# dev-wei/recman

Hardware: AMD Instinct MI355X
Metric: examples/sec fwd+bwd, Criteo-shape batch 65536; % HBM and MFMA roofline (higher is better)
Workload: dtype f32; 1 GPU; deepfm (BASELINE configs[1]); batch_per_gpu=65536, batch_all_gpus=65536, sparse_fields=26, rows_per_field=1000001, dense_fields=13, emb_dim=16, indices=uniform, table_row_loads=cached (rm_deepfm_step), row_gradient_stores=cached (as in fit(): the optimizer step gathers them next), optimizer_step=excluded, matrix_arithmetic=f32 MFMA (v_mfma_f32_16x16x4_f32), fp32 accumulate, hipgraph=True, table=single GPU

## Files before the change

recman_amd/build.py:

```python
import glob
import os
import shutil
import subprocess
import sys

CSRC = os.path.join(os.path.dirname(os.path.abspath(__file__)), "csrc")
LIB = os.path.join(CSRC, "librecman_hip.so")
ARCH = "gfx950"


def sources():
    return sorted(glob.glob(os.path.join(CSRC, "*.hip")))


def _stale():
    if not os.path.exists(LIB):
        return True
    t = os.path.getmtime(LIB)
    deps = sources() + glob.glob(os.path.join(CSRC, "*.h")) + glob.glob(
        os.path.join(CSRC, "..", "..", "include", "*.h"))
    return any(os.path.getmtime(p) > t for p in deps)


def hipcc():
    exe = shutil.which("hipcc") or "/opt/rocm/bin/hipcc"
    if not os.path.exists(exe):
        raise RuntimeError("hipcc not found: cannot build librecman_hip.so")
    return exe


def clean_experiments(verbose=True):
    for p in glob.glob(os.path.join(CSRC, "librecman_*.so")):
        if os.path.abspath(p) != os.path.abspath(LIB):
            if verbose:
                print(f"[build] removing stray experiment build {p}", flush=True)
            os.remove(p)


def build(force=False, verbose=True, extra_flags=(), out=None, only=None):
    clean_experiments(verbose)
    if out is None and not force and not _stale():
        return LIB
    if out is not None:
        if only:
            build(force=False, verbose=verbose)
        return _build_variant(out, extra_flags, verbose, only)
    objs = []
    procs = []
    for src in sources():
        obj = src[:-4] + ".o"
        cmd = [hipcc(), "-O3", "-std=c++17", f"--offload-arch={ARCH}", "-fPIC", "-c", src, "-o", obj,
               "-Wall", "-Wno-unused-function", *extra_flags]
        if verbose:
            print(" ".join(cmd), flush=True)
        procs.append((src, subprocess.Popen(cmd)))
        objs.append(obj)
    for src, p in procs:
        if p.wait() != 0:
            raise RuntimeError(f"hipcc failed on {src}")
    cmd = [hipcc(), "-shared", "-fPIC", f"--offload-arch={ARCH}", *objs, "-o", LIB]
    if verbose:
        print(" ".join(cmd), flush=True)
    subprocess.check_call(cmd)
    return LIB


def _build_variant(out, extra_flags, verbose, only=None):
    out = os.path.abspath(out)
    os.makedirs(os.path.dirname(out), exist_ok=True)
    tag = os.path.splitext(os.path.basename(out))[0]
    objs, procs = [], []
    for src in sources():
        if only and os.path.basename(src)[:-4] not in only:
            objs.append(src[:-4] + ".o")
            continue
        obj = os.path.join(os.path.dirname(out), f"{tag}_{os.path.basename(src)[:-4]}.o")
        cmd = [hipcc(), "-O3", "-std=c++17", f"--offload-arch={ARCH}", "-fPIC", "-c", src, "-o", obj,
               "-Wall", "-Wno-unused-function", *extra_flags]
        if verbose:
            print(" ".join(cmd), flush=True)
        procs.append((src, subprocess.Popen(cmd)))
        objs.append(obj)
    for src, p in procs:
        if p.wait() != 0:
            raise RuntimeError(f"hipcc failed on {src}")
    subprocess.check_call([hipcc(), "-shared", "-fPIC", f"--offload-arch={ARCH}", *objs, "-o", out])
    return out


if __name__ == "__main__":
    argv = sys.argv[1:]
    out = argv[argv.index("--out") + 1] if "--out" in argv else None
    flags = [a for a in argv if a.startswith("-D")]
    only = argv[argv.index("--only") + 1].split(",") if "--only" in argv else None
    print(build(force="--force" in argv, out=out, extra_flags=flags, only=only))
```

recman_amd/csrc/step.hip:

```cpp
#include "mlp_internal.h"
#include "rm_common.h"

namespace {

typedef float f32x4 __attribute__((ext_vector_type(4)));
typedef unsigned u32x4 __attribute__((ext_vector_type(4)));
typedef __amdgpu_buffer_rsrc_t rsrc_t;

constexpr int kWorkers = 7;
constexpr int kSlots = 4;
constexpr int kMaxF = 26;
constexpr int kRing = 3;
constexpr int kSlotB = 1024;
constexpr int kXBufB = kMaxF * kSlotB;
constexpr int kPartH = 0, kPartS = 2048, kPartQ = 3072, kPartSd = 3328, kPartB = 3584;
constexpr int kLDT = 36;
constexpr int kPubDh = 0, kPubDT = 2048, kPubGS = kPubDT + 16 * kLDT * 4, kPubG = kPubGS + 1024, kPubB = kPubG + 256;
constexpr int oX = 0;
constexpr int oDense = oX + kRing * kXBufB;
constexpr int oJunk = oDense + 4 * kSlotB;
constexpr int oPart = oJunk + kSlotB;
constexpr int oPub = oPart + 2 * kWorkers * kPartB;
constexpr int kRowB = 28 * 64;
constexpr int oRow = oPub + 2 * kPubB;
constexpr int oHT = oRow + 2 * kRowB;
constexpr int oD1T = oHT + 16 * 32 * 4;
constexpr int oY = oD1T + 16 * 32 * 4;
constexpr int oW1 = oY + 4 * 16 * 4;
constexpr int oPar = oW1 + 32 * 32 * 4;
constexpr int kParB0 = 0, kParB1 = 128, kParWo = 256, kParWd = 384, kParFo = 448;
constexpr int kLdsBytes = oPar + 448 + 28 * 4;
static_assert(kLdsBytes <= 160 * 1024, "LDS map exceeds a CU");

#ifndef RM_STEP_ABL
#define RM_STEP_ABL 0
#endif
#ifdef RM_STEP_STAMP
__device__ unsigned long long rm_step_stamp_buf[256 * 8 * 8];
#define ST_NOW() __builtin_amdgcn_s_memtime()
#define ST_DECL unsigned long long st_acc[8] = {0, 0, 0, 0, 0, 0, 0, 0}, st_t = ST_NOW(), st_t0 = st_t
#define ST_ADD(i) { const unsigned long long st_n = ST_NOW(); st_acc[i] += st_n - st_t; st_t = st_n; }
#define ST_FLUSH(wv) if (lane == 0 && blockIdx.x < 256) { st_acc[7] = ST_NOW() - st_t0; for (int i_ = 0; i_ < 8; ++i_) rm_step_stamp_buf[(blockIdx.x * 8 + (wv)) * 8 + i_] = st_acc[i_]; }
#else
#define ST_DECL
#define ST_ADD(i)
#define ST_FLUSH(wv)
#endif

struct StepArgs {
  const int64_t *idx, *field_off;
  const char *table;
  int64_t row_bytes;
  const float *dense;
  const int64_t *y;
  const float *y_f;
  const float *W0, *b0, *W1, *b1, *w_out, *w0_out, *lin_wd, *lin_w0;
  int F, Dn, H0, H1, act, task, Kp;
  float grad_scale;
  int64_t B;
  float *d_rows, *logit, *pred, *dlogit, *dW0_part, *sg_part, *loss_part;
  int packed, out_row_bytes, out_rows;
  const float *lin_mask;
};

__device__ __forceinline__ float act_slope(int act) {
  return act == RM_ACT_RELU ? 0.f : (act == RM_ACT_LEAKY_RELU ? 0.2f : 1.f);
}
__device__ __forceinline__ float actf(float v, float slope) { return v > 0.f ? v : slope * v; }
__device__ __forceinline__ float actg(float o, float slope) { return o > 0.f ? 1.f : slope; }

__device__ __forceinline__ int slot_field(int w, int j) {
  return j < 3 ? 7 * j + w : (w < 3 ? 21 + w : (w > 3 ? 20 + w : -1));
}

__device__ __forceinline__ f32x4 mfma16(float a, float b, f32x4 c) {
  return __builtin_amdgcn_mfma_f32_16x16x4f32(a, b, c, 0, 0, 0);
}
__device__ __forceinline__ f32x4 mfma16w(float a, float b, f32x4 c) {
  if (RM_STEP_ABL & 16) { c.x += a * b; return c; }
  return __builtin_amdgcn_mfma_f32_16x16x4f32(a, b, c, 0, 0, 0);
}

__device__ __forceinline__ int swz(int r) { return ((r >> 3) & 1) * 3; }

template <bool NT>
__device__ __forceinline__ void dma16(const char *src, char *lds_dst) {
  __builtin_amdgcn_global_load_lds((const __attribute__((address_space(1))) void *)src,
                                   (__attribute__((address_space(3))) void *)lds_dst, 16, 0, NT ? 2 : 0);
}

__device__ __forceinline__ void wait_vm(int younger) {
#define RM_WV(N) case N: asm volatile("s_waitcnt vmcnt(" #N ")" ::: "memory"); break;
  switch (younger) {
    RM_WV(24) RM_WV(23) RM_WV(22) RM_WV(21) RM_WV(20) RM_WV(19) RM_WV(18) RM_WV(17) RM_WV(16) RM_WV(15) RM_WV(14) RM_WV(13) RM_WV(12) RM_WV(11) RM_WV(10) RM_WV(9) RM_WV(8) RM_WV(7) RM_WV(6)
    RM_WV(5) RM_WV(4) RM_WV(3) RM_WV(2) RM_WV(1)
    default: asm volatile("s_waitcnt vmcnt(0)" ::: "memory"); break;
  }
#undef RM_WV
}

__device__ __forceinline__ float sum_q(float v) {
  {
    float a = v, c = v;
    asm("s_nop 1\n\tv_permlane16_swap_b32 %0, %1" : "+v"(a), "+v"(c));
    v = a + c;
  }
  {
    float a = v, c = v;
    asm("s_nop 1\n\tv_permlane32_swap_b32 %0, %1" : "+v"(a), "+v"(c));
    v = a + c;
  }
  return v;
}
__device__ __forceinline__ float sum_n(float v) {
#pragma unroll
  for (int o = 1; o < 16; o <<= 1) v += __shfl_xor(v, o, 64);
  return v;
}

template <bool NT, bool NT_OUT, bool PACKED>
__device__ __forceinline__ void step_worker(const StepArgs &a, char *smem, const int w, const int lane, const int T) {
  const int n = lane & 15, q = lane >> 4;
  const int F = a.F, H0 = a.H0, K = 16 * F + a.Dn;
  int fld[kSlots];
  bool sv[kSlots], sx[kSlots];
  float w0f[kSlots][2][4];
  float w0x[kSlots][2][4];
  f32x4 dw[kSlots][2];
#pragma unroll
  for (int j = 0; j < kSlots; ++j) {
    const int f = slot_field(w, j);
    sv[j] = f >= 0 && (f < F || (f == F && a.Dn > 0));
    sx[j] = f >= 0 && f < F;
    fld[j] = sv[j] ? f : 0;
    const int kb = 16 * fld[j];
#pragma unroll
    for (int uh = 0; uh < 2; ++uh) {
#pragma unroll
      for (int e = 0; e < 4; ++e) {
        const int kf = kb + 4 * q + e, uf = 16 * uh + n;
        const bool okf = sv[j] && kf < K && uf < H0;
        const float vf = a.W0[okf ? (int64_t)kf * H0 + uf : 0];
        w0f[j][uh][e] = okf ? vf : 0.f;
        const int kx = kb + n, ux = 16 * uh + 4 * q + e;
        const bool okx = sx[j] && kx < K && ux < H0;
        const float vx = a.W0[okx ? (int64_t)kx * H0 + ux : 0];
        w0x[j][uh][e] = okx ? vx : 0.f;
      }
      dw[j][uh] = f32x4{0.f, 0.f, 0.f, 0.f};
    }
  }
  const int64_t tstride = gridDim.x;
  const int lo_slice = n * 64 + 16 * (q ^ swz(n));
  int lo_col[4];
#pragma unroll
  for (int es = 0; es < 4; ++es) lo_col[es] = (4 * es + q) * 64 + 16 * ((n >> 2) ^ swz(4 * es + q)) + 4 * (n & 3);
  const int lo_row = n * F * 64 + 16 * q;
  auto slot_base = [&](int j, int tile) {
    const int ring = oX + ((tile + 6) % 3) * kXBufB + fld[j] * kSlotB, dn = oDense + (tile & 3) * kSlotB;
    return __builtin_amdgcn_readfirstlane((sx[j] || !sv[j]) ? ring : dn);
  };
  const int piece = 16 * ((lane & 3) ^ swz(lane >> 2));
  const int side_off = 64 + 4 * (lane & 1);
  float sdv[kSlots];
#pragma unroll
  for (int j = 0; j < kSlots; ++j) sdv[j] = 0.f;
  unsigned rp[4][kSlots];
  float lmask[kSlots];
#pragma unroll
  for (int j = 0; j < kSlots; ++j) {
    rp[0][j] = rp[1][j] = rp[2][j] = rp[3][j] = 0;
    lmask[j] = (PACKED && a.lin_mask != nullptr && sx[j]) ? a.lin_mask[fld[j]] : 1.f;
  }
  ST_DECL;
  ST_ADD(0);

  for (int s = -2; s <= T + 1; ++s) {
    const bool hasB = s - 2 >= 0 && s - 2 < T;
    const bool hasD = s + 1 >= 0 && s + 1 < T;
    float side_sum = 0.f;
#pragma unroll
    for (int j = 0; j < kSlots; ++j) side_sum += sx[j] ? sdv[j] : 0.f;
    {
      const int tb = s - 2, td = s + 1;
      const char *pub = smem + oPub + (tb & 1) * kPubB;
      char *xd = smem + oX + ((td + 3) % 3) * kXBufB;
      f32x4 dhB[2], gS, e4[kSlots];
      float dT[2][4], g, col[kSlots][4];
      if (hasB) {
#pragma unroll
        for (int j = 0; j < kSlots; ++j) {
          const char *xs = smem + slot_base(j, tb);
#pragma unroll
          for (int es = 0; es < 4; ++es)
            col[j][es] = *reinterpret_cast<const float *>(xs + lo_col[es]);
          e4[j] = *reinterpret_cast<const f32x4 *>(xs + lo_slice);
        }
#pragma unroll
        for (int uh = 0; uh < 2; ++uh) {
          dhB[uh] = *reinterpret_cast<const f32x4 *>(pub + kPubDh + (uh * 64 + lane) * 16);
#pragma unroll
          for (int es = 0; es < 4; ++es)
            dT[uh][es] = *reinterpret_cast<const float *>(pub + kPubDT + ((4 * es + q) * kLDT + 16 * uh + n) * 4);
        }
        gS = *reinterpret_cast<const f32x4 *>(pub + kPubGS + lane * 16);
        g = *reinterpret_cast<const float *>(pub + kPubG + lane * 4);
      }
      ST_ADD(1);
      unsigned rid[kSlots];
      if (PACKED) {
#pragma unroll
        for (int j = 0; j < kSlots; ++j) {
          rp[3][j] = rp[2][j];
          rp[2][j] = rp[1][j];
          rp[1][j] = rp[0][j];
        }
      }
      if (hasD) {
        const unsigned *rowid = reinterpret_cast<const unsigned *>(smem + oRow + (td & 1) * kRowB);
#pragma unroll
        for (int j = 0; j < kSlots; ++j) {
          rid[j] = rowid[fld[j] * 16 + (lane >> 2)];
          if (PACKED) rp[0][j] = rowid[fld[j] * 16 + n];
        }
      }
      asm volatile("s_waitcnt lgkmcnt(0)" ::: "memory");
      const int64_t ex0 = ((int64_t)blockIdx.x + tb * tstride) * 16;
      const int64_t left = a.B - ex0;
      const int rows_t = left < 16 ? (int)left : 16;
      const rsrc_t rd = PACKED ? __builtin_amdgcn_make_buffer_rsrc(a.d_rows, 0, hasB ? a.out_rows * a.out_row_bytes : 0, 0x00020000)
                               : __builtin_amdgcn_make_buffer_rsrc(a.d_rows + (hasB ? ex0 * F * 16 : 0), 0,
                                                                   hasB ? rows_t * F * 64 : 0, 0x00020000);
      const bool ex_ok = n < rows_t;
      auto store_row = [&](int i, const f32x4 &o) {
        const bool ok = sx[i] && !(RM_STEP_ABL & 2);
        if (PACKED) {
          const int base = (ok && ex_ok) ? (int)rp[3][i] * a.out_row_bytes : 0x7ffffff0 - 64;
          __builtin_amdgcn_raw_buffer_store_b128(__builtin_bit_cast(u32x4, o), rd, base + 16 * q, 0, NT_OUT ? 2 : 0);
          const f32x4 tail = f32x4{g, g * lmask[i], 0.f, 0.f};
          __builtin_amdgcn_raw_buffer_store_b128(__builtin_bit_cast(u32x4, tail), rd, q == 0 ? base + 64 : 0x7ffffff0,
                                                 0, NT_OUT ? 2 : 0);
        } else {
          const int off = lo_row + __builtin_amdgcn_readfirstlane(ok ? fld[i] * 64 : 0x70000000);
          __builtin_amdgcn_raw_buffer_store_b128(__builtin_bit_cast(u32x4, o), rd, off, 0, NT_OUT ? 2 : 0);
        }
      };
      f32x4 acc[kSlots];
#pragma unroll
      for (int j = 0; j < kSlots; ++j) {
        if (hasD) {
          const char *row = a.table + ((RM_STEP_ABL & 4) || !sx[j] ? 0 : (int64_t)rid[j] * a.row_bytes);
          if (!(RM_STEP_ABL & 8)) dma16<NT>(row + piece, sx[j] ? xd + fld[j] * kSlotB : smem + oJunk);
          if (!(RM_STEP_ABL & 1)) sdv[j] = *reinterpret_cast<const float *>(row + side_off);
        }
        __builtin_amdgcn_sched_barrier(0);
        if (hasB) {
          acc[j] = f32x4{0.f, 0.f, 0.f, 0.f};
#pragma unroll
          for (int es = 0; es < 4; ++es) {
            dw[j][0] = mfma16w(col[j][es], dT[0][es], dw[j][0]);
            dw[j][1] = mfma16w(col[j][es], dT[1][es], dw[j][1]);
            acc[j] = mfma16w(w0x[j][0][es], dhB[0][es], acc[j]);
            acc[j] = mfma16w(w0x[j][1][es], dhB[1][es], acc[j]);
          }
        }
        __builtin_amdgcn_sched_barrier(0);
        if (hasB && j > 0) {
          const int i = j - 1;
          f32x4 o;
          o.x = acc[i].x + (gS.x - g * e4[i].x);
          o.y = acc[i].y + (gS.y - g * e4[i].y);
          o.z = acc[i].z + (gS.z - g * e4[i].z);
          o.w = acc[i].w + (gS.w - g * e4[i].w);
          store_row(i, o);
        }
      }
      if (hasB) {
        const int i = kSlots - 1;
        f32x4 o;
        o.x = acc[i].x + (gS.x - g * e4[i].x);
        o.y = acc[i].y + (gS.y - g * e4[i].y);
        o.z = acc[i].z + (gS.z - g * e4[i].z);
        o.w = acc[i].w + (gS.w - g * e4[i].w);
        store_row(i, o);
      }
    }
    ST_ADD(6);
    if (s >= 0 && s < T) {
      constexpr int SP = PACKED ? 2 : 1;
      const int younger = 1 + ((s - 3 >= 0) ? 2 * SP : 0) + 8 * (hasD ? 1 : 0) + 4 * SP * (hasB ? 1 : 0);
      wait_vm(younger);
      ST_ADD(3);
      f32x4 acc0 = f32x4{0.f, 0.f, 0.f, 0.f}, acc1 = acc0, S = acc0, Q = acc0;
      f32x4 x4[kSlots];
#pragma unroll
      for (int j = 0; j < kSlots; ++j) {
        x4[j] = *reinterpret_cast<const f32x4 *>(smem + slot_base(j, s) + lo_slice);
      }
#pragma unroll
      for (int j = 0; j < kSlots; ++j) {
#pragma unroll
        for (int ks = 0; ks < 4; ++ks) {
          acc0 = mfma16w(w0f[j][0][ks], x4[j][ks], acc0);
          acc1 = mfma16w(w0f[j][1][ks], x4[j][ks], acc1);
        }
        const float m = sx[j] ? 1.f : 0.f;
        S += m * x4[j];
        Q += m * (x4[j] * x4[j]);
      }
      char *part = smem + oPart + ((s & 1) * kWorkers + w) * kPartB;
      *reinterpret_cast<f32x4 *>(part + kPartH + lane * 16) = acc0;
      *reinterpret_cast<f32x4 *>(part + kPartH + (64 + lane) * 16) = acc1;
      *reinterpret_cast<f32x4 *>(part + kPartS + lane * 16) = S;
      *reinterpret_cast<float *>(part + kPartQ + lane * 4) = (Q.x + Q.y) + (Q.z + Q.w);
      *reinterpret_cast<float *>(part + kPartSd + lane * 4) = side_sum;
    }
    ST_ADD(4);
    __syncthreads();
    ST_ADD(5);
  }
#pragma unroll
  for (int j = 0; j < kSlots; ++j)
    if (sv[j]) {
#pragma unroll
      for (int uh = 0; uh < 2; ++uh)
#pragma unroll
        for (int i = 0; i < 4; ++i)
          a.dW0_part[((int64_t)blockIdx.x * a.Kp + 16 * fld[j] + 4 * q + i) * 32 + 16 * uh + n] = dw[j][uh][i];
    }
  ST_ADD(0);
  ST_FLUSH(w);
}

__device__ __forceinline__ void step_head(const StepArgs &a, char *smem, const int lane, const int T) {
  const int n = lane & 15, q = lane >> 4;
  const int F = a.F, Dn = a.Dn, H0 = a.H0, H1 = a.H1;
  const float act = act_slope(a.act);
  const int64_t B = a.B, tstride = gridDim.x;
  {
    float *w1s = reinterpret_cast<float *>(smem + oW1);
#pragma unroll
    for (int i = 0; i < 16; ++i) {
      const int e = lane + 64 * i, u = e >> 5, v = e & 31;
      const bool ok = u < H0 && v < H1;
      const float f = a.W1[ok ? u * H1 + v : 0];
      w1s[u * 32 + 4 * ((v >> 2) ^ (u & 7)) + (v & 3)] = ok ? f : 0.f;
    }
    float *par = reinterpret_cast<float *>(smem + oPar);
    if (lane < 32) {
      const float f0 = a.b0[lane < H0 ? lane : 0], f1 = a.b1[lane < H1 ? lane : 0], f2 = a.w_out[lane < H1 ? lane : 0];
      par[kParB0 / 4 + lane] = lane < H0 ? f0 : 0.f;
      par[kParB1 / 4 + lane] = lane < H1 ? f1 : 0.f;
      par[kParWo / 4 + lane] = lane < H1 ? f2 : 0.f;
      const float f3 = a.lin_wd[lane < Dn ? lane : 0];
      if (lane < 16) par[kParWd / 4 + lane] = lane < Dn ? f3 : 0.f;
      if (lane < 28) reinterpret_cast<unsigned *>(par)[kParFo / 4 + lane] = (unsigned)a.field_off[lane < F ? lane : F - 1];
    }
  }
  const float *w1s = reinterpret_cast<const float *>(smem + oW1);
  const char *par = smem + oPar;
  const float w0o = a.w0_out[0], lw0 = a.lin_w0[0];

  f32x4 dW1[2][2];
  float db0[2][4], db1[2][4], dwo[2][4], dxd[4], sg = 0.f, loss_acc = 0.f;
#pragma unroll
  for (int x = 0; x < 2; ++x)
#pragma unroll
    for (int i = 0; i < 4; ++i) {
      dW1[x][0][i] = dW1[x][1][i] = 0.f;
      db0[x][i] = db1[x][i] = dwo[x][i] = 0.f;
    }
#pragma unroll
  for (int i = 0; i < 4; ++i) dxd[i] = 0.f;

  auto ex_of = [&](int t) {
    const int64_t b = ((int64_t)blockIdx.x + t * tstride) * 16 + n;
    return b < B ? b : B - 1;
  };
  unsigned idr[7];
  float dnr[4];
  unsigned yr = 0;
#pragma unroll
  for (int j = 0; j < 7; ++j) idr[j] = 0;
#pragma unroll
  for (int i = 0; i < 4; ++i) dnr[i] = 0.f;
  auto load_ids = [&](int t) {
    const unsigned *p = reinterpret_cast<const unsigned *>(a.idx + ex_of(t) * F);
#pragma unroll
    for (int j = 0; j < 7; ++j) idr[j] = p[2 * (q + 4 * j < F ? q + 4 * j : F - 1)];
  };
  if (T > 0) load_ids(0);
  ST_DECL;
  ST_ADD(0);

  for (int s = -2; s <= T + 1; ++s) {
    if (s - 1 >= 0 && s - 1 < T) {
      const int t = s - 1;
      const int64_t bex = ((int64_t)blockIdx.x + t * tstride) * 16 + n;
      const bool valid = bex < B;
      f32x4 pre[2], S = f32x4{0.f, 0.f, 0.f, 0.f};
      pre[0] = pre[1] = S;
      float ss = 0.f, y1 = 0.f, ls = 0.f;
#pragma unroll
      for (int w = 0; w < kWorkers; ++w) {
        const char *part = smem + oPart + ((t & 1) * kWorkers + w) * kPartB;
        pre[0] += *reinterpret_cast<const f32x4 *>(part + kPartH + lane * 16);
        pre[1] += *reinterpret_cast<const f32x4 *>(part + kPartH + (64 + lane) * 16);
        S += *reinterpret_cast<const f32x4 *>(part + kPartS + lane * 16);
        ss += *reinterpret_cast<const float *>(part + kPartQ + lane * 4);
        const float2 sd = *reinterpret_cast<const float2 *>(part + kPartSd + 16 * n);
        y1 += sd.x;
        ls += sd.y;
        if (w == 3) __builtin_amdgcn_sched_barrier(0);
      }
      const f32x4 dn4 = Dn > 0 ? *reinterpret_cast<const f32x4 *>(smem + oDense + (t & 3) * kSlotB + n * 64 + 16 * (q ^ swz(n)))
                               : f32x4{0.f, 0.f, 0.f, 0.f};
      const f32x4 wdv = *reinterpret_cast<const f32x4 *>(par + kParWd + 16 * q);
      const float fmq = sum_q(S.x * S.x + S.y * S.y + S.z * S.z + S.w * S.w - ss);
      const float lind = sum_q(dn4.x * wdv.x + dn4.y * wdv.y + dn4.z * wdv.z + dn4.w * wdv.w);
      const float fm = y1 + 0.5f * fmq;
      const float lin = ls + lind + lw0;
      const float ty = *reinterpret_cast<const float *>(smem + oY + ((t & 3) * 16 + n) * 4);
      ST_ADD(1);
      float h0[2][4], h1[2][4];
#pragma unroll
      for (int h = 0; h < 2; ++h) {
        const f32x4 b0v = *reinterpret_cast<const f32x4 *>(par + kParB0 + (16 * h + 4 * q) * 4);
#pragma unroll
        for (int i = 0; i < 4; ++i) h0[h][i] = actf(pre[h][i] + b0v[i], act);
        *reinterpret_cast<f32x4 *>(smem + oHT + (n * 32 + 16 * h + 4 * q) * 4) =
            f32x4{h0[h][0], h0[h][1], h0[h][2], h0[h][3]};
      }
      f32x4 acc[2];
      acc[0] = acc[1] = f32x4{0.f, 0.f, 0.f, 0.f};
#pragma unroll
      for (int uh = 0; uh < 2; ++uh)
#pragma unroll
        for (int i = 0; i < 4; ++i) {
          const int u = 16 * uh + 4 * q + i;
          const float a0 = w1s[u * 32 + 4 * ((n >> 2) ^ (u & 7)) + (n & 3)];
          const float a1 = w1s[u * 32 + 4 * ((4 + (n >> 2)) ^ (u & 7)) + (n & 3)];
          acc[0] = mfma16(a0, h0[uh][i], acc[0]);
          acc[1] = mfma16(a1, h0[uh][i], acc[1]);
        }
      float dnn = 0.f;
      f32x4 wov[2];
#pragma unroll
      for (int h = 0; h < 2; ++h) {
        const f32x4 b1v = *reinterpret_cast<const f32x4 *>(par + kParB1 + (16 * h + 4 * q) * 4);
        wov[h] = *reinterpret_cast<const f32x4 *>(par + kParWo + (16 * h + 4 * q) * 4);
#pragma unroll
        for (int i = 0; i < 4; ++i) {
          h1[h][i] = actf(acc[h][i] + b1v[i], act);
          dnn += h1[h][i] * wov[h][i];
        }
      }
      dnn = sum_q(dnn) + w0o;
      float z = 0.f;
      z += lin;
      z += fm;
      z += dnn;
      float p, dz;
      const float lt = rm_loss_point(z, ty, a.task, &p, &dz);
      float gb = dz * (1.0f / (float)B);
      gb *= a.grad_scale;
      gb = valid ? gb : 0.f;
      if (valid && q == 0) {
        a.logit[bex] = z;
        a.pred[bex] = p;
        a.dlogit[bex] = gb;
        loss_acc += lt;
      }
      ST_ADD(2);
      float dh1[2][4], dh0[2][4];
#pragma unroll
      for (int h = 0; h < 2; ++h) {
#pragma unroll
        for (int i = 0; i < 4; ++i) dh1[h][i] = gb * wov[h][i] * actg(h1[h][i], act);
        *reinterpret_cast<f32x4 *>(smem + oD1T + (n * 32 + 16 * h + 4 * q) * 4) =
            f32x4{dh1[h][0], dh1[h][1], dh1[h][2], dh1[h][3]};
      }
      acc[0] = acc[1] = f32x4{0.f, 0.f, 0.f, 0.f};
#pragma unroll
      for (int vh = 0; vh < 2; ++vh) {
        const f32x4 c0 = *reinterpret_cast<const f32x4 *>(w1s + n * 32 + 4 * ((4 * vh + q) ^ (n & 7)));
        const f32x4 c1 = *reinterpret_cast<const f32x4 *>(w1s + (16 + n) * 32 + 4 * ((4 * vh + q) ^ (n & 7)));
#pragma unroll
        for (int i = 0; i < 4; ++i) {
          acc[0] = mfma16(c0[i], dh1[vh][i], acc[0]);
          acc[1] = mfma16(c1[i], dh1[vh][i], acc[1]);
        }
      }
      char *pub = smem + oPub + (t & 1) * kPubB;
#pragma unroll
      for (int h = 0; h < 2; ++h) {
#pragma unroll
        for (int i = 0; i < 4; ++i) dh0[h][i] = acc[h][i] * actg(h0[h][i], act);
        const f32x4 d4 = f32x4{dh0[h][0], dh0[h][1], dh0[h][2], dh0[h][3]};
        *reinterpret_cast<f32x4 *>(pub + kPubDh + (h * 64 + lane) * 16) = d4;
        *reinterpret_cast<f32x4 *>(pub + kPubDT + (n * kLDT + 16 * h + 4 * q) * 4) = d4;
      }
      *reinterpret_cast<f32x4 *>(pub + kPubGS + lane * 16) = f32x4{gb * S.x, gb * S.y, gb * S.z, gb * S.w};
      *reinterpret_cast<float *>(pub + kPubG + lane * 4) = gb;
      ST_ADD(3);
#pragma unroll
      for (int es = 0; es < 4; ++es) {
        float av[2], bv[2];
#pragma unroll
        for (int h = 0; h < 2; ++h) {
          av[h] = *reinterpret_cast<const float *>(smem + oHT + ((4 * es + q) * 32 + 16 * h + n) * 4);
          bv[h] = *reinterpret_cast<const float *>(smem + oD1T + ((4 * es + q) * 32 + 16 * h + n) * 4);
        }
#pragma unroll
        for (int uh = 0; uh < 2; ++uh)
#pragma unroll
          for (int vh = 0; vh < 2; ++vh) dW1[uh][vh] = mfma16(av[uh], bv[vh], dW1[uh][vh]);
      }
#pragma unroll
      for (int h = 0; h < 2; ++h)
#pragma unroll
        for (int i = 0; i < 4; ++i) {
          db0[h][i] += dh0[h][i];
          db1[h][i] += dh1[h][i];
          dwo[h][i] += gb * h1[h][i];
        }
      sg += q == 0 ? gb : 0.f;
      dxd[0] += gb * dn4.x;
      dxd[1] += gb * dn4.y;
      dxd[2] += gb * dn4.z;
      dxd[3] += gb * dn4.w;
    }
    ST_ADD(4);
    if (s + 1 >= 0 && s + 1 < T) {
      const int t = s + 1;
      if (Dn > 0)
        *reinterpret_cast<f32x4 *>(smem + oDense + (t & 3) * kSlotB + n * 64 + 16 * (q ^ swz(n))) =
            f32x4{4 * q + 0 < Dn ? dnr[0] : 0.f, 4 * q + 1 < Dn ? dnr[1] : 0.f, 4 * q + 2 < Dn ? dnr[2] : 0.f,
                  4 * q + 3 < Dn ? dnr[3] : 0.f};
      if (q == 0)
        *reinterpret_cast<float *>(smem + oY + ((t & 3) * 16 + n) * 4) = a.y ? (float)(int)yr : __uint_as_float(yr);
    }
    if (s + 2 < T) {
      unsigned *rowid = reinterpret_cast<unsigned *>(smem + oRow + ((s + 2) & 1) * kRowB);
#pragma unroll
      for (int j = 0; j < 7; ++j)
        rowid[(q + 4 * j) * 16 + n] = idr[j] + *reinterpret_cast<const unsigned *>(par + kParFo + (q + 4 * j) * 4);
    }
    __builtin_amdgcn_sched_barrier(0);
    if (s + 2 >= 0 && s + 2 < T) {
      const int64_t b = ex_of(s + 2);
      if (Dn > 0) {
        const float *dp = a.dense + b * Dn;
#pragma unroll
        for (int i = 0; i < 4; ++i) dnr[i] = dp[4 * q + i < Dn ? 4 * q + i : 0];
      }
      const unsigned *yp = a.y ? reinterpret_cast<const unsigned *>(a.y + b) : reinterpret_cast<const unsigned *>(a.y_f + b);
      yr = *yp;
    }
    if (s + 3 < T) load_ids(s + 3);
    ST_ADD(6);
    __syncthreads();
    ST_ADD(5);
  }

  float *sgp = a.sg_part + (int64_t)blockIdx.x * kRmSgStride;
#pragma unroll
  for (int uh = 0; uh < 2; ++uh)
#pragma unroll
    for (int vh = 0; vh < 2; ++vh)
#pragma unroll
      for (int i = 0; i < 4; ++i) sgp[(16 * uh + 4 * q + i) * 32 + 16 * vh + n] = dW1[uh][vh][i];
#pragma unroll
  for (int h = 0; h < 2; ++h)
#pragma unroll
    for (int i = 0; i < 4; ++i) {
      const float s0 = sum_n(db0[h][i]), s1 = sum_n(db1[h][i]), s2 = sum_n(dwo[h][i]);
      if (n == 0) {
        const int u = 16 * h + 4 * q + i;
        sgp[2 * 1024 + u] = s0;
        sgp[2 * 1024 + 32 + u] = s1;
        sgp[2 * 1024 + 64 + u] = s2;
      }
    }
#pragma unroll
  for (int i = 0; i < 4; ++i) {
    const float sx = sum_n(dxd[i]);
    if (n == 0) sgp[kRmSgDense + 4 * q + i] = sx;
  }
  const float sgt = rm_wave_sum(sg), lst = rm_wave_sum(loss_acc);
  if (lane == 0) {
    sgp[2 * 1024 + 64 + 32] = sgt;
    a.loss_part[blockIdx.x] = lst;
  }
  ST_ADD(0);
  ST_FLUSH(7);
}

template <bool NT, bool NT_OUT, bool PACKED>
__global__ __launch_bounds__(512) void deepfm_step_kernel(StepArgs a) {
  extern __shared__ __attribute__((aligned(16))) char smem[];
  const int lane = threadIdx.x & 63;
  const int wave = __builtin_amdgcn_readfirstlane(threadIdx.x >> 6);
  const int64_t ntiles = (a.B + 15) / 16;
  const int T = (int)((ntiles - blockIdx.x + gridDim.x - 1) / gridDim.x);
#ifndef RM_STEP_PRIO
#define RM_STEP_PRIO 1
#endif
  if (wave < kWorkers) {
    if (RM_STEP_PRIO == 1 && wave >= 4) __builtin_amdgcn_s_setprio(1);
    step_worker<NT, NT_OUT, PACKED>(a, smem, wave, lane, T);
  } else {
    if (RM_STEP_PRIO) __builtin_amdgcn_s_setprio(2);
    step_head(a, smem, lane, T);
  }
}

}

#ifdef RM_STEP_STAMP
extern "C" int rm_debug_step_stamps(unsigned long long *host, int n) {
  return (int)hipMemcpyFromSymbol(host, HIP_SYMBOL(rm_step_stamp_buf), sizeof(unsigned long long) * n);
}
#endif

extern "C" int64_t rm_deepfm_step_workspace(int F, int Dn) {
  const int Kp = ((16 * F + Dn + 63) / 64) * 64;
  return (int64_t)256 * Kp * 32 + (int64_t)256 * kRmSgStride + 256;
}

extern "C" int rm_deepfm_step_supported(int F, int D, int64_t table_ld, int Dn, int NL, const int *H) {
  if (D != 16 || table_ld < 20 || table_ld % 4 != 0 || F < 1 || F > 26 || Dn < 0 || Dn > 16 || NL != 2 || !H) return 0;
  return H[0] >= 1 && H[0] <= 32 && H[1] >= 1 && H[1] <= 32;
}

extern "C" int rm_deepfm_step(const int64_t *idx, const float *table, int64_t table_ld, const int64_t *field_off,
                              const float *dense, int Dn, const int64_t *y, const float *y_f, int64_t B, int F,
                              int D, int NL, const int *H, const float *const *W, const float *const *bias,
                              const float *w_out, const float *w0_out, const float *lin_w_dense,
                              const float *lin_w0, int act, int task, float grad_scale, float *d_rows,
                              float *logit, float *pred, float *dlogit, float *loss, float *const *dW,
                              float *const *db, float *d_w_out, float *d_w0_out, float *d_lin_w_dense,
                              float *d_lin_w0, float *workspace, int64_t packed_rows, const float *lin_field_mask,
                              int flags, rm_stream_t stream) {
  RM_REQUIRE(H && rm_deepfm_step_supported(F, D, table_ld, Dn, NL, H),
             "rm_deepfm_step: needs D = 16, fused rows (table_ld >= 20, a multiple of 4), F <= 26, Dn <= 16 and two "
             "hidden layers of width <= 32");
  RM_REQUIRE(B >= 0, "rm_deepfm_step: B < 0");
  if (B == 0) return RM_OK;
  RM_REQUIRE(idx && table && field_off && (Dn == 0 || (dense && lin_w_dense)) && W && bias && W[0] && W[1] &&
                 bias[0] && bias[1] && w_out && w0_out && lin_w0 && d_rows && logit && pred && dlogit && loss && dW &&
                 dW[0] && dW[1] && workspace,
             "rm_deepfm_step: NULL argument");
  RM_REQUIRE((y != nullptr) != (y_f != nullptr), "rm_deepfm_step: exactly one of y / y_f");
  RM_REQUIRE(task == 0 || task == 1, "rm_deepfm_step: task must be 0 or 1");
  RM_REQUIRE(rm_aligned16(table) && rm_aligned16(d_rows), "rm_deepfm_step: table / d_rows must be 16-byte aligned");
  RM_REQUIRE(packed_rows >= 0 && packed_rows * 80 < (1ll << 31), "rm_deepfm_step: packed_rows out of range");
  const int K = 16 * F + Dn, Kp = ((K + 63) / 64) * 64;
  const int64_t ntiles = (B + 15) / 16;
  const int nblk = rm_grid_cap(ntiles, 256);
  StepArgs a;
  a.idx = idx; a.field_off = field_off; a.table = reinterpret_cast<const char *>(table); a.row_bytes = table_ld * 4;
  a.dense = dense; a.y = y; a.y_f = y_f;
  a.W0 = W[0]; a.b0 = bias[0]; a.W1 = W[1]; a.b1 = bias[1]; a.w_out = w_out; a.w0_out = w0_out;
  a.lin_wd = Dn > 0 ? lin_w_dense : w_out; a.lin_w0 = lin_w0;
  a.F = F; a.Dn = Dn; a.H0 = H[0]; a.H1 = H[1]; a.act = act; a.task = task; a.Kp = Kp;
  a.grad_scale = grad_scale; a.B = B;
  a.d_rows = d_rows; a.logit = logit; a.pred = pred; a.dlogit = dlogit;
  a.packed = packed_rows > 0; a.out_row_bytes = 80; a.out_rows = (int)packed_rows; a.lin_mask = lin_field_mask;
  a.dW0_part = workspace;
  a.sg_part = workspace + (int64_t)256 * Kp * 32;
  a.loss_part = a.sg_part + (int64_t)256 * kRmSgStride;
  hipStream_t st = (hipStream_t)stream;
  const bool nt = (flags & 1) != 0, nt_out = (flags & 2) != 0;
#define RM_STEP(NT_, NTO_, PK_)                                                                              \
  {                                                                                                          \
    (void)hipFuncSetAttribute(reinterpret_cast<const void *>(deepfm_step_kernel<NT_, NTO_, PK_>),            \
                              hipFuncAttributeMaxDynamicSharedMemorySize, kLdsBytes);                        \
    hipLaunchKernelGGL((deepfm_step_kernel<NT_, NTO_, PK_>), dim3(nblk), dim3(512), kLdsBytes, st, a);       \
  }
  if (a.packed) {
    if (nt) RM_STEP(true, false, true) else RM_STEP(false, false, true)
  } else if (nt) {
    if (nt_out) RM_STEP(true, true, false) else RM_STEP(true, false, false)
  } else {
    if (nt_out) RM_STEP(false, true, false) else RM_STEP(false, false, false)
  }
#undef RM_STEP
  RM_CHECK_LAUNCH("rm_deepfm_step");
  if (flags & 4) return RM_OK;
  return rm_internal_mlp_finish(a.dW0_part, nblk, K, Kp, H[0], dW[0], a.sg_part, nblk, 2, H, dW, db, d_w_out,
                                d_w0_out, Dn > 0 ? d_lin_w_dense : nullptr, d_lin_w0, Dn, a.loss_part, nblk, B, loss,
                                st);
}
```

Measured before the change: 632.0 million examples/s.

## Fetch side-entry scalars via LDS DMA and peel pipeline loop in step worker

Replaces the per-slot scalar global load of each row's side value (offset 64) with 4-byte global_load_lds DMAs into a new per-worker LDS entry buffer, issued between MFMA slots during the forward phase. The pipelined segment loop is peeled into prologue, steady-state and epilogue calls with compile-time hasB/hasD flags, and vmcnt waits are recomputed. __syncthreads is swapped for an explicit lgkmcnt wait plus s_barrier, and hipFuncSetAttribute is cached per device so it does not run on every launch. This adds LDS usage and more complex wait-count bookkeeping, which risks subtle ordering bugs.

Result: slower. 622.2 million examples/s (-1.6%).

```diff
diff --git a/recman_amd/build.py b/recman_amd/build.py
--- a/recman_amd/build.py
+++ b/recman_amd/build.py
@@ -7,6 +7,7 @@
 CSRC = os.path.join(os.path.dirname(os.path.abspath(__file__)), "csrc")
 LIB = os.path.join(CSRC, "librecman_hip.so")
 ARCH = "gfx950"
+CFLAGS = ["-O3", "-std=c++17", f"--offload-arch={ARCH}", "-fPIC", "-Wall", "-Wno-unused-function"]
 
 
 def sources():
@@ -49,8 +50,7 @@
     procs = []
     for src in sources():
         obj = src[:-4] + ".o"
-        cmd = [hipcc(), "-O3", "-std=c++17", f"--offload-arch={ARCH}", "-fPIC", "-c", src, "-o", obj,
-               "-Wall", "-Wno-unused-function", *extra_flags]
+        cmd = [hipcc(), *CFLAGS, "-c", src, "-o", obj, *extra_flags]
         if verbose:
             print(" ".join(cmd), flush=True)
         procs.append((src, subprocess.Popen(cmd)))
@@ -75,8 +75,7 @@
             objs.append(src[:-4] + ".o")
             continue
         obj = os.path.join(os.path.dirname(out), f"{tag}_{os.path.basename(src)[:-4]}.o")
-        cmd = [hipcc(), "-O3", "-std=c++17", f"--offload-arch={ARCH}", "-fPIC", "-c", src, "-o", obj,
-               "-Wall", "-Wno-unused-function", *extra_flags]
+        cmd = [hipcc(), *CFLAGS, "-c", src, "-o", obj, *extra_flags]
         if verbose:
             print(" ".join(cmd), flush=True)
         procs.append((src, subprocess.Popen(cmd)))
diff --git a/recman_amd/csrc/step.hip b/recman_amd/csrc/step.hip
--- a/recman_amd/csrc/step.hip
+++ b/recman_amd/csrc/step.hip
@@ -1,3 +1,5 @@
+#include <atomic>
+
 #include "mlp_internal.h"
 #include "rm_common.h"
 
@@ -29,7 +31,8 @@
 constexpr int oW1 = oY + 4 * 16 * 4;
 constexpr int oPar = oW1 + 32 * 32 * 4;
 constexpr int kParB0 = 0, kParB1 = 128, kParWo = 256, kParWd = 384, kParFo = 448;
-constexpr int kLdsBytes = oPar + 448 + 28 * 4;
+constexpr int oEnt = oPar + 448 + 28 * 4;
+constexpr int kLdsBytes = oEnt + kWorkers * 2 * 256;
 static_assert(kLdsBytes <= 160 * 1024, "LDS map exceeds a CU");
 
 #ifndef RM_STEP_ABL
@@ -88,6 +91,10 @@
   __builtin_amdgcn_global_load_lds((const __attribute__((address_space(1))) void *)src,
                                    (__attribute__((address_space(3))) void *)lds_dst, 16, 0, NT ? 2 : 0);
 }
+__device__ __forceinline__ void dma4(const char *src, char *lds_dst) {
+  __builtin_amdgcn_global_load_lds((const __attribute__((address_space(1))) void *)src,
+                                   (__attribute__((address_space(3))) void *)lds_dst, 4, 0, 0);
+}
 
 __device__ __forceinline__ void wait_vm(int younger) {
 #define RM_WV(N) case N: asm volatile("s_waitcnt vmcnt(" #N ")" ::: "memory"); break;
@@ -97,6 +104,14 @@
     default: asm volatile("s_waitcnt vmcnt(0)" ::: "memory"); break;
   }
 #undef RM_WV
+}
+
+template <bool HEAD>
+__device__ __forceinline__ void tile_barrier() {
+  if (HEAD)
+    asm volatile("s_waitcnt lgkmcnt(0)\n\ts_barrier ; tile barrier (head)" ::: "memory");
+  else
+    asm volatile("s_waitcnt lgkmcnt(0)\n\ts_barrier ; tile barrier (worker)" ::: "memory");
 }
 
 __device__ __forceinline__ float sum_q(float v) {
@@ -161,10 +176,9 @@
     return __builtin_amdgcn_readfirstlane((sx[j] || !sv[j]) ? ring : dn);
   };
   const int piece = 16 * ((lane & 3) ^ swz(lane >> 2));
-  const int side_off = 64 + 4 * (lane & 1);
-  float sdv[kSlots];
-#pragma unroll
-  for (int j = 0; j < kSlots; ++j) sdv[j] = 0.f;
+  char *ent = smem + oEnt + w * 512;
+  const int ent_ex = (lane >> 1) & 15, ent_off = 64 + 4 * (lane & 1);
+  const int ent_rd = 4 * (2 * (lane >> 2) + (lane & 1));
   unsigned rp[4][kSlots];
   float lmask[kSlots];
 #pragma unroll
@@ -175,12 +189,7 @@
   ST_DECL;
   ST_ADD(0);
 
-  for (int s = -2; s <= T + 1; ++s) {
-    const bool hasB = s - 2 >= 0 && s - 2 < T;
-    const bool hasD = s + 1 >= 0 && s + 1 < T;
-    float side_sum = 0.f;
-#pragma unroll
-    for (int j = 0; j < kSlots; ++j) side_sum += sx[j] ? sdv[j] : 0.f;
+  auto segment = [&](const int s, const bool hasB, const bool hasD, const bool fwd) __attribute__((always_inline)) {
     {
       const int tb = s - 2, td = s + 1;
       const char *pub = smem + oPub + (tb & 1) * kPubB;
@@ -251,7 +260,6 @@
         if (hasD) {
           const char *row = a.table + ((RM_STEP_ABL & 4) || !sx[j] ? 0 : (int64_t)rid[j] * a.row_bytes);
           if (!(RM_STEP_ABL & 8)) dma16<NT>(row + piece, sx[j] ? xd + fld[j] * kSlotB : smem + oJunk);
-          if (!(RM_STEP_ABL & 1)) sdv[j] = *reinterpret_cast<const float *>(row + side_off);
         }
         __builtin_amdgcn_sched_barrier(0);
         if (hasB) {
@@ -286,11 +294,26 @@
       }
     }
     ST_ADD(6);
-    if (s >= 0 && s < T) {
+    auto entry = [&](int p) __attribute__((always_inline)) {
+      if (hasD && !(RM_STEP_ABL & 1)) {
+        const bool hi = lane >= 32;
+        const int f = hi ? fld[2 * p + 1] : fld[2 * p];
+        const bool x = hi ? sx[2 * p + 1] : sx[2 * p];
+        const unsigned rid = *reinterpret_cast<const unsigned *>(smem + oRow + ((s + 1) & 1) * kRowB + (f * 16 + ent_ex) * 4);
+        asm volatile("s_waitcnt lgkmcnt(0)" ::: "memory");
+        dma4(a.table + (int64_t)((RM_STEP_ABL & 4) || !x ? 0u : rid) * a.row_bytes + ent_off, ent + 256 * p);
+      }
+    };
+    if (fwd) {
       constexpr int SP = PACKED ? 2 : 1;
-      const int younger = 1 + ((s - 3 >= 0) ? 2 * SP : 0) + 8 * (hasD ? 1 : 0) + 4 * SP * (hasB ? 1 : 0);
-      wait_vm(younger);
+      wait_vm((hasD && !(RM_STEP_ABL & 8) ? 4 : 0) + (hasB ? 4 * SP : 0));
       ST_ADD(3);
+      float side_sum = 0.f;
+#pragma unroll
+      for (int j = 0; j < kSlots; ++j) {
+        const float e = *reinterpret_cast<const float *>(ent + 256 * (j >> 1) + 128 * (j & 1) + ent_rd);
+        side_sum += sx[j] ? e : 0.f;
+      }
       f32x4 acc0 = f32x4{0.f, 0.f, 0.f, 0.f}, acc1 = acc0, S = acc0, Q = acc0;
       f32x4 x4[kSlots];
 #pragma unroll
@@ -307,6 +330,11 @@
         const float m = sx[j] ? 1.f : 0.f;
         S += m * x4[j];
         Q += m * (x4[j] * x4[j]);
+        if (j & 1) {
+          __builtin_amdgcn_sched_barrier(0);
+          entry(j >> 1);
+          __builtin_amdgcn_sched_barrier(0);
+        }
       }
       char *part = smem + oPart + ((s & 1) * kWorkers + w) * kPartB;
       *reinterpret_cast<f32x4 *>(part + kPartH + lane * 16) = acc0;
@@ -314,10 +342,27 @@
       *reinterpret_cast<f32x4 *>(part + kPartS + lane * 16) = S;
       *reinterpret_cast<float *>(part + kPartQ + lane * 4) = (Q.x + Q.y) + (Q.z + Q.w);
       *reinterpret_cast<float *>(part + kPartSd + lane * 4) = side_sum;
+    } else {
+      entry(0);
+      entry(1);
     }
     ST_ADD(4);
-    __syncthreads();
+    tile_barrier<false>();
     ST_ADD(5);
+  };
+  if (T >= 4) {
+    segment(-2, false, false, false);
+    segment(-1, false, true, false);
+    segment(0, false, true, true);
+    segment(1, false, true, true);
+#pragma clang loop unroll(disable)
+    for (int s = 2; s <= T - 2; ++s) segment(s, true, true, true);
+    segment(T - 1, true, false, true);
+    segment(T, true, false, false);
+    segment(T + 1, true, false, false);
+  } else {
+#pragma clang loop unroll(disable)
+    for (int s = -2; s <= T + 1; ++s) segment(s, s - 2 >= 0 && s - 2 < T, s + 1 >= 0 && s + 1 < T, s >= 0 && s < T);
   }
 #pragma unroll
   for (int j = 0; j < kSlots; ++j)
@@ -393,6 +438,7 @@
   ST_DECL;
   ST_ADD(0);
 
+#pragma clang loop unroll(disable)
   for (int s = -2; s <= T + 1; ++s) {
     if (s - 1 >= 0 && s - 1 < T) {
       const int t = s - 1;
@@ -559,7 +605,7 @@
     }
     if (s + 3 < T) load_ids(s + 3);
     ST_ADD(6);
-    __syncthreads();
+    tile_barrier<true>();
     ST_ADD(5);
   }
 
@@ -613,6 +659,18 @@
     if (RM_STEP_PRIO) __builtin_amdgcn_s_setprio(2);
     step_head(a, smem, lane, T);
   }
+}
+
+template <bool NT, bool NT_OUT, bool PACKED>
+void step_raise_lds_limit() {
+  static std::atomic<unsigned long long> done{0};
+  int dev = 0;
+  if (hipGetDevice(&dev) != hipSuccess) dev = 64;
+  const unsigned long long bit = dev < 64 ? 1ull << dev : 0;
+  if (bit && (done.load(std::memory_order_acquire) & bit)) return;
+  (void)hipFuncSetAttribute(reinterpret_cast<const void *>(deepfm_step_kernel<NT, NT_OUT, PACKED>),
+                            hipFuncAttributeMaxDynamicSharedMemorySize, kLdsBytes);
+  done.fetch_or(bit, std::memory_order_release);
 }
 
 }
@@ -674,8 +732,7 @@
   const bool nt = (flags & 1) != 0, nt_out = (flags & 2) != 0;
 #define RM_STEP(NT_, NTO_, PK_)                                                                              \
   {                                                                                                          \
-    (void)hipFuncSetAttribute(reinterpret_cast<const void *>(deepfm_step_kernel<NT_, NTO_, PK_>),            \
-                              hipFuncAttributeMaxDynamicSharedMemorySize, kLdsBytes);                        \
+    step_raise_lds_limit<NT_, NTO_, PK_>();                                                                  \
     hipLaunchKernelGGL((deepfm_step_kernel<NT_, NTO_, PK_>), dim3(nblk), dim3(512), kLdsBytes, st, a);       \
   }
   if (a.packed) {
```
